# mfouda/epsilon

Hardware: AMD Instinct MI355X
Metric: ADMM iters/sec, dense Lasso 1e4x5e4 (higher is better)
Workload: dtype f32

## Files before the change

### epsilon_amd/csrc/capi.cc

```cpp
#include "../../include/epsilon_hip.h"

#include <algorithm>
#include <cmath>
#include <cstdio>
#include <cstdlib>
#include <cstring>
#include <map>
#include <memory>
#include <set>
#include <string>
#include <vector>

#include "admm.h"
#include "block.h"
#include "comm.h"
#include "kernels.h"
#include "linear_map.h"
#include "wire.h"

using namespace eps;

struct eps_result {
  std::string status;
  std::vector<std::string> ids;
  std::vector<HostArray> values;
};

struct eps_solver {
  std::shared_ptr<DataMap> data;
  std::unique_ptr<Solver> solver;
// ... 263 lines not shown
    } else if (std::strcmp(key, "fused") == 0) {
      setenv("EPSILON_HIP_FUSED", value, 1);
    } else if (std::strcmp(key, "batch_wide") == 0) {
      if (std::strcmp(value, "0") != 0 && std::strcmp(value, "1") != 0)
        EPS_FATAL("batch_wide must be 0 or 1, got " << value);
      setenv("EPSILON_HIP_BATCH_WIDE", value, 1);
    } else if (std::strcmp(key, "fused_matrix") == 0) {
      bool ok = false;
      for (const char* v : {"0", "pass", "wide", "auto"}) ok = ok || std::strcmp(value, v) == 0;
      if (!ok) EPS_FATAL("fused_matrix must be 0, pass, wide or auto, got " << value);
      setenv("EPSILON_HIP_FUSED_MATRIX", value, 1);
    } else if (std::strcmp(key, "fused_zero") == 0) {
      if (std::strcmp(value, "0") != 0 && std::strcmp(value, "auto") != 0)
        EPS_FATAL("fused_zero must be 0 or auto, got " << value);
      setenv("EPSILON_HIP_FUSED_ZERO", value, 1);
    } else if (std::strcmp(key, "refine") == 0) {
      if (std::strcmp(value, "auto") == 0) unsetenv("EPSILON_HIP_REFINE");
      else setenv("EPSILON_HIP_REFINE", value, 1);
    } else {
      EPS_FATAL("unknown option " << key);
    }
  });
}

int eps_device_count(void) {
  int count = 0;
  if (hipGetDeviceCount(&count) != hipSuccess) {
    (void)hipGetLastError();
    return 0;
  }
// ... 467 lines not shown
    const void* src = device_ptr;
    if (src == nullptr) {
      own = Synthetic(static_cast<int64_t>(bytes / 4), F32, 1.0);
      src = own.data();
    }
    EPS_HIP(hipDeviceSynchronize());
    DVec dst;
    if (mode == 2) dst = DVec::Empty(static_cast<int64_t>(bytes / 4), F32);
    if (grid <= 0) grid = 2048;
    DVec scratch = DVec::Empty(grid, F32);
    *ms_avg = TimeLaunches(iters, [&] {
      k::StreamProbe(mode, src, mode == 2 ? dst.data() : nullptr, static_cast<int64_t>(bytes),
                     scratch.as<float>(), grid);
    });
    (void)rt;
  });
}

int eps_bench_gemm(int trans_a, int trans_b, int64_t M, int64_t N, int64_t K, int lower_only,
                   int iters, double* ms_avg) {
  return Guard([&] {
    const DType dt = ConfiguredDType();
    const bool rnd = std::getenv("EPSILON_HIP_BENCH_RANDOM") != nullptr;
    auto operand = [&](int64_t count, uint64_t seed) {
      if (!rnd) return Synthetic(count, dt, 1.0);
      DVec v = DVec::Empty(count, dt);
      k::FillHash(v, seed);
      return v;
    };
    DVec A = operand(M * K, 0xA11CEull);
// ... 328 lines not shown
```

### epsilon_amd/csrc/fused_route.cc

```cpp
#include "fused_route.h"

#include <algorithm>
#include <cmath>
#include <cstdlib>
#include <cstring>
#include <map>

#include "admm.h"
#include "comm.h"
#include "kernels.h"

namespace eps {
namespace {


template <class Record>
void SetThreshold(Record* s, const ScaledZoneDesc& z, double a1) {
  s->alpha_vec = z.alpha_vec;
  s->beta_vec = z.beta_vec;
  s->Bs = z.Bs;
  s->Cs = z.Cs;
  s->a1 = a1;
  s->lam = z.lam;
  s->alpha = z.alpha;
// ... 72 lines not shown
  for (const StateSlice& s : table) s.home->Set(s.key, s.v);
}
std::vector<BlockVector*> Homes(const MultiBlockParts& a) {
  std::vector<BlockVector*> h = {&a.u};
  for (auto* c : {&a.x, &a.y, &a.y_prev})
    for (BlockVector& v : *c) h.push_back(&v);
  return h;
}

bool FusedDisabled() {
  const char* env = std::getenv("EPSILON_HIP_FUSED");
  return env && env[0] == '0';
}

int BatchWideMin();

constexpr int64_t kMatrixFusedMinRows = 256;

enum MatrixRoute { kMatrixOff, kMatrixAuto, kMatrixPass, kMatrixWide };
MatrixRoute FusedMatrixMode() {
  const char* e = std::getenv("EPSILON_HIP_FUSED_MATRIX");
  if (e == nullptr || std::strcmp(e, "auto") == 0) return kMatrixAuto;
  if (std::strcmp(e, "0") == 0) return kMatrixOff;
  if (std::strcmp(e, "pass") == 0) return kMatrixPass;
  if (std::strcmp(e, "wide") == 0) return kMatrixWide;
  EPS_FATAL("fused_matrix must be 0, pass, wide or auto, got " << e);
}

constexpr int64_t kZeroFusedMinRows = 256;

// ... 68 lines not shown
  DVec state_all, snapshot;
  DVec norm_work;
  int norm_slot = 0;
  bool whiten = false;
  double wscale = 1;
  DVec X, Ahat, rhat;
  k::LassoFusedArgs pass;
  int64_t cols = 1;
  bool group = false;
  int64_t group_rows = 0;
  bool wide = false;
  bool rhs_aligned = true;
  std::vector<k::LassoInstance> members;
  DVec table;
  WideSweep ws;

  bool Enable(const MultiBlockParts& a) {
    if (FusedDisabled() || a.prox.size() != 2 || a.num_constraints != 1 || !a.b.data().empty()) return false;
    const ShardSpec& sh = ShardSpec::Get();
    if (sh.active() && sh.consensus_terms()) return false;
    if (!a.prox[0]->DescribeLeastSquares(&ls)) return false;
    cols = ls.cols;
    const MatrixRoute matrix_mode = cols > 1 ? FusedMatrixMode() : kMatrixAuto;
    if (cols > 1 && (matrix_mode == kMatrixOff || sh.active())) return false;
    if (!a.prox[1]->DescribeScaledZone(&sz)) {
      GroupNorm2Desc gn;
      if (cols == 1 || !a.prox[1]->DescribeGroupNorm2(&gn) || gn.cols != cols) return false;
      group = true;
      group_rows = gn.rows;
      sz = ScaledZoneDesc();
// ... 198 lines not shown
    } else if (cols == 1) {
      inv.Apply();
    } else if (inv.packed.n > 0) {
      k::SymvPackedBatch(m, inv.D->scale(), inv.packed, table, static_cast<int>(cols), inv.work);
    } else {
      for (int64_t c = 0; c < cols; ++c) inv.Column(c).Apply();
    }
  }

  void BuildPass() {
    const DenseMatrixImpl& L = *ls.L_arg_var;
    pass.m = m;
    pass.n = n;
    pass.lda = whiten ? m : L.rows();
    pass.A = whiten ? Ahat : L.data();
    k::LassoInstance& s = pass.inst;
    s.w = w;
    s.tpart = tpart;
    s.p = whiten ? w : p;
    s.rhs = whiten ? rhat : ls.rhs_arg;
    s.kappa = -L.scale() * (whiten ? wscale : 1.0);
    s.pkappa = -L.scale();
    SetThreshold(&s, sz, a1);
    if (cols == 1) return;
    members.assign(static_cast<size_t>(cols), s);
    rhs_aligned = true;
    for (int64_t c = 0; c < cols; ++c) {
      k::LassoInstance& mb = members[static_cast<size_t>(c)];
      auto col = [&](const DVec& v, int64_t len) { return v.n > 0 ? v.Slice(c * len, len) : v; };
      mb.w = col(s.w, m);
// ... 16 lines not shown
    const int K = static_cast<int>(cols);
    const double* group_lam = group ? &sz.lam : nullptr;
    if (wide) {
      constexpr int PW = WideSweep::PW;
      for (int first = 0; first < K; first += PW) {
        const int nk = std::min(PW, K - first);
        const uint64_t live = nk == 64 ? ~uint64_t(0) : (uint64_t(1) << nk) - 1;
        const int64_t off = static_cast<int64_t>(first) * m;
        ws.Run(table, first, nk, live, w.Slice(off, ws.panel_len), whiten ? DVec() : p.Slice(off, ws.panel_len),
               group_lam);
      }
      return;
    }
    const int width = k::LassoBatchWidth(m, n, dt);
    for (int first = 0; first < K; first += width)
      k::LassoBatchPass(m, n, pass.lda, pass.A, table, first, std::min(width, K - first), group_lam);
    k::ReducePartialsBatch(m, grid, table, K, dt, rhs_aligned);
    if (!whiten) ApplyInverseFixed();
  }

  void Sweep() override {
    if (cols > 1) {
      MatrixSweep();
    } else if (use_peer) {
      pass.epoch = Runtime::Get().peer()->view().epoch;
      k::LassoFusedPass(pass);
      ForwardTailPeer();
    } else {
      k::LassoFusedPass(pass);
      ForwardTail(true);
    }
// ... 151 lines not shown
      return &views[first];
    };
    grid = k::LassoFusedGrid(m, n, dt);
    w = DVec::Zeros(m, dt);
    p = DVec::Zeros(m, dt);
    tpart = DVec::Empty(static_cast<int64_t>(grid) * m, dt);
    inv.Init(zp.Dinv_arg, m, p, w, a.shared_cache);
    {
      const StateSlice* sn = side(n, zp.x_constraint_key, ix, sx.var_key, zp.x_key, &state_n);
      pass.m = m;
      pass.n = n;
      pass.lda = L.rows();
      pass.A = L.data();
      pass.chain = 2;
      pass.e0 = sn[6].v;
      k::LassoInstance& s = pass.inst;
      s.w = w;
      s.tpart = tpart;
      s.p = p;
      s.rhs = zp.rhs_arg;
      s.u = sn[0].v;
      s.x1 = sn[1].v;
      s.x0 = sn[2].v;
      s.y1 = sn[3].v;
      s.y0 = sn[4].v;
      s.y1prev = sn[5].v;
      s.kappa = s.pkappa = -L.scale();
      SetThreshold(&s, sx, ax);
    }
    if (has_z) {
// ... 87 lines not shown
    for (BlockVector* home : {&a.x, &a.z, &a.u, &a.z_prev})
      for (const std::string& key : {ls.var_key, sz.var_key})
        views.push_back({home, key, DVec::Zeros(n, dt), home != &a.z_prev});
    const DVec &x0 = views[0].v, &x1 = views[1].v, &z0 = views[2].v, &z1 = views[3].v, &u0 = views[4].v,
               &u1 = views[5].v, &z0p = views[6].v, &z1p = views[7].v;
    p = DVec::Zeros(m, dt);
    w = DVec::Zeros(m, dt);
    grid = k::LassoFusedGrid(m, n, dt);
    tpart = DVec::Empty(static_cast<int64_t>(grid) * m, dt);
    pass.m = m;
    pass.n = n;
    pass.lda = L.rows();
    pass.A = L.data();
    pass.chain = 1;
    pass.a0 = a0;
    pass.e0 = u1;
    pass.e1 = z1p;
    k::LassoInstance& s = pass.inst;
    s.w = w;
    s.tpart = tpart;
    s.u = u0;
    s.x0 = x0;
    s.x1 = x1;
    s.y0 = z0;
    s.y1 = z1;
    s.y1prev = z0p;
    s.p = p;
    s.rhs = ls.rhs_arg;
    s.kappa = s.pkappa = -L.scale();
    SetThreshold(&s, sz, a1);
// ... 10 lines not shown
    k::LassoFusedPass(pass);
    k::ReducePartials(m, grid, tpart, pass.inst.pkappa, 0.0, p, ls.rhs_arg.n != 0 ? &ls.rhs_arg : nullptr);
    ls.Dinv_arg->Apply(1.0, p, 0.0, w);
  }
};

template <class Route, class Parts>
std::unique_ptr<FusedRoute> Recognise(const Parts& parts) {
  std::unique_ptr<Route> r(new Route);
  if (!r->Enable(parts)) return nullptr;
  return std::unique_ptr<FusedRoute>(std::move(r));
}

}

std::unique_ptr<FusedRoute> RecogniseMultiBlockRoute(const MultiBlockParts& parts) {
  const bool zero = FusedZeroAuto();
  if (auto r = Recognise<LassoRoute>(parts)) return r;
  return zero ? Recognise<ZeroRoute>(parts) : nullptr;
}

std::unique_ptr<FusedRoute> RecogniseTwoBlockRoute(const TwoBlockParts& parts) {
  return Recognise<TwoBlockRoute>(parts);
}

namespace {

struct BatchMember {
  Solver* solver;
  LassoRoute* route;
// ... 33 lines not shown
void RunFusedGroup(const Group& g) {
  const double t0 = Now();
  const LassoRoute& lead = *g[0].route;
  const DType dt = lead.dt;
  SetCurrentDType(dt);
  const int64_t m = lead.m, n = lead.n;
  const int width = k::LassoBatchWidth(m, n, dt);
  const DVec& P = lead.inv.packed;
  bool rhs_aligned = true;
  for (const BatchMember& b : g) {
    const DVec& rhs = b.route->pass.inst.rhs;
    if (rhs.n > 0) rhs_aligned = rhs_aligned && reinterpret_cast<uintptr_t>(rhs.data()) % 16 == 0;
  }
  const int K = static_cast<int>(g.size());
  DVec symv_work = P.n > 0 ? DVec::Empty(K * k::SymvWorkspace(m), dt) : DVec();

  std::vector<int> active(K);
  for (int i = 0; i < K; ++i) active[i] = i;
  DVec table;
  auto upload = [&] {
    std::vector<const k::LassoInstance*> v;
    for (int i : active) v.push_back(&g[i].route->pass.inst);
    k::LassoBatchUpload(v, dt, &table);
  };
  upload();
  auto sweep = [&] {
    const int na = static_cast<int>(active.size());
    for (int first = 0; first < na; first += width)
      k::LassoBatchPass(m, n, lead.pass.lda, lead.pass.A, table, first, std::min(width, na - first));
    k::ReducePartialsBatch(m, lead.grid, table, na, dt, rhs_aligned);
    if (lead.whiten) {
    } else if (P.n > 0) {
      k::SymvPackedBatch(m, lead.inv.D->scale(), P, table, na, symv_work);
    } else {
      for (int i : active) g[i].route->inv.Apply();
    }
  };
  RunGroupSchedule(g, t0, &active, sweep, [&](const std::vector<int>&) {
    if (!active.empty()) upload();
  });
}

bool BatchWideEnabled() {
  const char* e = std::getenv("EPSILON_HIP_BATCH_WIDE");
// ... 96 lines not shown
```

### epsilon_amd/csrc/fused_route.h

```cpp
#pragma once

#include <memory>
#include <vector>

#include "block.h"
#include "prox.h"

namespace eps {

class FusedRoute {
 public:
  virtual ~FusedRoute() {}
  virtual void Sweep() = 0;

  virtual bool HasCheck() const { return false; }
  virtual bool PipelineChecks() const { return false; }
  virtual void LaunchNorms() {}
  struct Check {
    double r = 0, s = 0;
    double max_norm = 0;
    double atu = 0;
  };
  virtual Check FinishCheck() { return Check(); }
  virtual void SaveSnapshot() {}
// ... 9 lines not shown
  const BlockVector& b;
  const std::vector<std::unique_ptr<ProxOperator>>& prox;
  DataMap* data;
  OpCache* shared_cache;
  BlockVector& u;
  std::vector<BlockVector>&x, &y, &y_prev;
};
struct TwoBlockParts {
  int num_constraints;
  const AffineOperator& constr_H;
  const std::vector<std::unique_ptr<ProxOperator>>& prox;
  DataMap* data;
  BlockVector &x, &z, &u, &z_prev;
};

std::unique_ptr<FusedRoute> RecogniseMultiBlockRoute(const MultiBlockParts& parts);
std::unique_ptr<FusedRoute> RecogniseTwoBlockRoute(const TwoBlockParts& parts);

}
```

### epsilon_amd/csrc/kernels.h

```cpp
#pragma once

#include "device.h"

namespace eps {
struct PeerView;
namespace k {

void Fill(const DVec& y, double v);
void Copy(const DVec& dst, const DVec& src);
void FillHash(const DVec& y, uint64_t seed);
void Axpby(const DVec& y, double a, const DVec& x, double b);
void DiagMul(const DVec& y, double a, const DVec& d, const DVec& x, double b);
void ConvertFromF64(const DVec& dst, const double* src_dev);
void ConvertToF64(double* dst_dev, const DVec& src);
void ConvertFromF32(const DVec& dst, const float* src_dev);

void SumSq(const DVec& x, double* slot, bool accumulate);
void SumSqDiff(const DVec& x, const DVec& y, double* slot, bool accumulate);
void Dot(const DVec& x, const DVec& y, double* slot, bool accumulate);

void Gemv(bool trans, int64_t rows, int64_t cols, double alpha, const DVec& A, int64_t lda,
          const DVec& x, double beta, const DVec& y);

void Symv(int64_t n, double alpha, const DVec& S, int64_t lds, const DVec& x, double beta,
// ... 14 lines not shown
  DVec alpha_vec, beta_vec;
  DVec p, rhs;
  double kappa = 0;
  double Bs = 0, Cs = 0, a1 = 0;
  double lam = 0, alpha = 1, beta = 1, M = 0;
  double pkappa = 0;
};
struct LassoFusedArgs {
  int64_t m = 0, n = 0, lda = 0;
  DVec A;
  LassoInstance inst;
  unsigned* epoch = nullptr;
  int chain = 0;
  double a0 = 1;
  DVec e0, e1;
};

enum SmoothFn { SMOOTH_EXP, SMOOTH_LOGISTIC, SMOOTH_NEG_ENTR, SMOOTH_INV_POS, SMOOTH_NEG_LOG };

struct ZeroRowsArgs {
  int64_t m = 0;
  int nparts = 0;
  DVec w, tpart, r, rhs, g;
  DVec u, z, zq, yz, yq, yzprev, yqprev;
  DVec alpha_vec, beta_vec;
  double e = 0, pkappa = 0;
  double Bs = 0, Cs = 0, a1 = 0, lam = 0, alpha = 1, beta = 1, M = 0;
  bool smooth = false;
  SmoothFn fn = SMOOTH_LOGISTIC;
  DVec hs, hys, hv;
};
void ZeroFusedRows(const ZeroRowsArgs& args);
void ZeroSmoothHead(const ZeroRowsArgs& args);
bool LassoFusedSupported(int64_t m, int64_t n, const DVec& A, int64_t lda);
int LassoFusedGrid(int64_t m, int64_t n, DType dt = F32);
int LassoFusedBlock(int64_t m, int64_t n, DType dt);
void LassoFusedPass(const LassoFusedArgs& args);
void LassoFusedNorms(const DVec& u, const DVec& y0, const DVec& y1, const DVec& y1prev, double* out6,
                     const DVec& work, const unsigned* peer_err = nullptr);

template <class T> struct LassoBatchInst {
  const T* w;
  T* tpart;
  T* u; T* x0; T* x1; T* y0; T* y1; T* y1prev;
  const T* alpha_v;
  const T* beta_v;
  T* p;
  const T* rhs;
  T kappa, Bs, Cs, a1, lam, alpha, beta, M;
  T pkappa;
};
int LassoBatchWidth(int64_t m, int64_t n, DType dt);
void LassoBatchUpload(const std::vector<const LassoInstance*>& members, DType dt, DVec* table);
void LassoBatchPass(int64_t m, int64_t n, int64_t lda, const DVec& A, const DVec& table, int first,
                    int count, const double* group_lam = nullptr);
void ReducePartialsBatch(int64_t m, int nparts, const DVec& table, int count, DType dt,
                         bool rhs_aligned);
void SymvPackedBatch(int64_t m, double alpha, const DVec& P, const DVec& table, int count,
                     const DVec& work);

constexpr int kLassoWidePanel = 64;
bool LassoWideSupported(int64_t m, int64_t n, const DVec& A, int64_t lda);
int LassoWideSlabs(int64_t m, int64_t n);
void LassoWideBack(int64_t m, int64_t n, int64_t lda, const DVec& A, const DVec& table, int first, int nk,
                   uint64_t active, const DVec& W, int64_t ldw, const DVec& V, int64_t ldv,
                   const double* group_lam = nullptr);
void LassoWideForward(int64_t m, int64_t n, int64_t lda, const DVec& A, int nk, const DVec& V, int64_t ldv,
                      const DVec& T, int64_t ldt);
void LassoWideReduce(int64_t m, int64_t n, const DVec& table, int first, int nk, uint64_t active, const DVec& T,
                     int64_t ldt);
// ... 14 lines not shown
                 bool lower_only = false, int64_t outer = 1, int64_t sA2 = 0, int64_t sB2 = 0);
void SymmetrizeFromLower(const DVec& C, int64_t n, int64_t ldc);
bool GemmSplitF16(bool transA, bool transB, int64_t M, int64_t N, int64_t K, double alpha, const DVec& A,
                  int64_t lda, const DVec& B, int64_t ldb, double beta, const DVec& C, int64_t ldc,
                  bool lower_only);
bool GemmF64Pipe(bool transA, bool transB, int64_t M, int64_t N, int64_t K, double alpha, const DVec& A,
                 int64_t lda, int64_t sA, const DVec& B, int64_t ldb, int64_t sB, double beta,
                 const DVec& C, int64_t ldc, int64_t sC, int64_t n1, int64_t batch, bool lower_only,
                 int64_t sA2, int64_t sB2);
bool GemmSplitF16KRange(int kmode, int64_t M, int64_t N, int64_t K, double alpha, const DVec& A, int64_t lda,
                        const DVec& B, int64_t ldb, const DVec& C, int64_t ldc);
bool SyrkSplitF16LowerTriangular(int64_t n, const DVec& X, int64_t ldx, const DVec& C, int64_t ldc);
bool MultiGemv(bool transA, int64_t M, int64_t N, int64_t K, double alpha, const DVec& A, int64_t lda,
               const DVec& B, int64_t ldb, double beta, const DVec& C, int64_t ldc);
void StreamProbe(int mode, const void* src, void* dst, int64_t bytes, float* scratch, int grid);

void MatCopy(bool trans, int64_t rows, int64_t cols, double alpha, const DVec& src,
             int64_t lds, const DVec& dst);
void AddDiag(const DVec& W, int64_t n, int64_t ld, double alpha, const DVec* d);
void ColAbsSums(const DVec& A, int64_t rows, int64_t cols, int64_t lda, double* colsum_dev);
void ScaleByInvNorm(const DVec& y, const DVec& x, const double* normsq_dev);
void KronDense(const DVec& dst, const DVec& A, int64_t mA, int64_t nA, const DVec& B,
               int64_t mB, int64_t nB);

void SpdInverseInPlace(const DVec& W, int64_t n, DVec* factor_inverse = nullptr);
void SetPotrfForm(int form);
void SpdInverseColumns(const DVec& W, int64_t n, int64_t lo, int64_t cnt, const DVec& Out);

struct ScaledZoneArgs {
  double lam = 0, alpha = 1, beta = 1, M = 0, C = 0;
// ... 56 lines not shown
```

### epsilon_amd/csrc/kernels_fused.hip

```cpp
#include <hip/hip_runtime.h>

#include <cstdlib>
#include <type_traits>

#include "kernels.h"
#include "kernels_fused_chain.h"

namespace eps {
namespace k {

namespace {

constexpr int kBlock = 256;

template <class T, int NR, int BS, int MODE>
__global__ __launch_bounds__(BS, 2) void LassoFusedStreamKernelT(
    int64_t m, int64_t n, const T* __restrict__ A, int64_t lda, const T* __restrict__ w,
    FusedScalarsT<T> c, T* u, T* x0, T* x1, T* y0, T* y1, T* y1prev, T* __restrict__ tpart,
    unsigned* epoch, T* e0, T* e1) {
  typedef typename Chunk<T>::V V;
  constexpr int R = Chunk<T>::R;
  __shared__ T red[2][BS / 64];
  if (epoch != nullptr && blockIdx.x == 0 && threadIdx.x == 0) *epoch += 1u;
  const int tid = threadIdx.x, lane = tid & 63, wave = tid >> 6;
  const V zero = T(0);
  V wv[NR], tp[NR];
  int64_t row[NR];
#pragma unroll
  for (int q = 0; q < NR; ++q) {
    row[q] = (static_cast<int64_t>(q) * BS + tid) * R;
    wv[q] = row[q] < m ? *reinterpret_cast<const V*>(w + row[q]) : zero;
    tp[q] = zero;
  }
  const int64_t npairs = (n + 1) / 2;
  auto column = [&](int64_t step) -> int64_t {
    const int64_t jp = blockIdx.x + (step >> 1) * gridDim.x;
    const int64_t j = 2 * jp + (step & 1);
    return (jp < npairs && j < n) ? j : -1;
  };
  auto load = [&](V (&a)[NR], int64_t j) {
    const T* cp = A + j * lda;
#pragma unroll
    for (int q = 0; q < NR; ++q) {
      if (row[q] < m) a[q] = __builtin_nontemporal_load(reinterpret_cast<const V*>(cp + row[q]));
      else a[q] = zero;
    }
  };
  V cur[NR], nxt[NR];
  int64_t step = 0;
  int64_t j = column(0);
  if (j >= 0) load(cur, j);
  int par = 0;
  while (j >= 0) {
    int64_t jn = column(step + 1);
    if (jn < 0 && ((step + 1) & 1)) jn = column(step + 2);
    const int64_t step_n = (jn >= 0 && column(step + 1) < 0) ? step + 2 : step + 1;
    if (jn >= 0) load(nxt, jn);
    const T uj = u[j], y0j = y0[j], y1j = y1[j];
    T u1j = T(0);
// ... 63 lines not shown
  T* out = tpart + static_cast<int64_t>(blockIdx.x) * m;
#pragma unroll
  for (int q = 0; q < NR; ++q)
    if (row[q] < m) *reinterpret_cast<V*>(out + row[q]) = tp[q];
}

template <class T, int NR, int BS>
void LaunchFused(const LassoFusedArgs& a, int grid) {
  const LassoBatchInst<T> i = Narrow<T>(a.inst);
  T* e0 = a.chain != 0 ? a.e0.as<T>() : nullptr;
  T* e1 = a.chain == 1 ? a.e1.as<T>() : nullptr;
  hipLaunchKernelGGL(
      (a.chain == 1 ? LassoFusedStreamKernelT<T, NR, BS, 1>
                    : a.chain == 2 ? LassoFusedStreamKernelT<T, NR, BS, 2> : LassoFusedStreamKernelT<T, NR, BS, 0>),
      dim3(grid), dim3(BS), 0, Runtime::Get().stream(), a.m, a.n, a.A.as<T>(), a.lda, i.w,
      ScalarsOf<T>(i, a.a0, a.inst.a1), i.u, i.x0, i.x1, i.y0, i.y1, i.y1prev, i.tpart, a.epoch, e0, e1);
}

template <class T>
void LaunchFusedT(const LassoFusedArgs& a, int grid, int block) {
  const int64_t need = (a.m + Chunk<T>::R * block - 1) / (Chunk<T>::R * block);
  if (block == 256) {
    if (need <= 1) LaunchFused<T, 1, 256>(a, grid);
    else if (need <= 2) LaunchFused<T, 2, 256>(a, grid);
    else if (need <= 4) LaunchFused<T, 4, 256>(a, grid);
    else if (need <= 8) LaunchFused<T, 8, 256>(a, grid);
    else LaunchFused<T, 10, 256>(a, grid);
    return;
  }
  if constexpr (std::is_same<T, float>::value) {
    if (need <= 2) return LaunchFused<T, 2, 512>(a, grid);
// ... 236 lines not shown

int LassoFusedGrid(int64_t m, int64_t n, DType dt) {
  int64_t npairs = (n + 1) / 2;
  const int64_t rows_per_chunk = dt == F32 ? 4 : 2;
  const bool one_per_cu = LassoFusedBlock(m, n, dt) == 512 && m > 512 * 5 * rows_per_chunk;
  int64_t g = one_per_cu ? 256 : 512;
  static const char* env = std::getenv("EPSILON_HIP_FUSED_GRID");
  if (env && std::atoi(env) > 0) g = std::atoi(env);
  if (g > npairs) g = npairs;
  if (g < 1) g = 1;
  const int64_t per = (npairs + g - 1) / g;
  g = (npairs + per - 1) / per;
  return static_cast<int>(g < 1 ? 1 : g);
}

void LassoFusedPass(const LassoFusedArgs& a) {
  EPS_CHECK(LassoFusedSupported(a.m, a.n, a.A, a.lda));
  const DType dt = a.A.dt;
  const LassoInstance& s = a.inst;
  EPS_CHECK(s.w.n == a.m && s.w.dt == dt);
  for (const DVec* v : {&s.u, &s.x0, &s.x1, &s.y0, &s.y1, &s.y1prev})
    EPS_CHECK(v->n == a.n && v->dt == dt);
  for (const DVec* v : {&s.alpha_vec, &s.beta_vec})
    if (v->n > 0) EPS_CHECK(v->n == a.n && v->dt == dt);
  if (a.chain == 1) EPS_CHECK(a.e0.n == a.n && a.e1.n == a.n && a.e0.dt == dt && a.e1.dt == dt);
  if (a.chain == 2) EPS_CHECK(a.e0.n == a.n && a.e0.dt == dt);
  const int grid = LassoFusedGrid(a.m, a.n, dt);
  const int block = LassoFusedBlock(a.m, a.n, dt);
  EPS_CHECK(s.tpart.n >= static_cast<int64_t>(grid) * a.m && s.tpart.dt == dt);
  EPS_CHECK(reinterpret_cast<uintptr_t>(s.w.data()) % 16 == 0 &&
            reinterpret_cast<uintptr_t>(s.tpart.data()) % 16 == 0);
  ProfScope prof(a.chain == 2 ? "zero_fused" : "lasso_fused", a.m, a.n);
  if (dt == F32) LaunchFusedT<float>(a, grid, block);
  else LaunchFusedT<double>(a, grid, block);
  EPS_HIP(hipGetLastError());
}

}
}
```

### epsilon_amd/csrc/kernels_fused_batch.hip

```cpp
#include <hip/hip_runtime.h>

#include <vector>

#include "kernels.h"
#include "kernels_fused_chain.h"

namespace eps {
namespace k {

namespace {

constexpr int kBlock = 256;

template <class T, int NR, int KB, bool GROUP>
__global__ __launch_bounds__(kBlock) void LassoBatchStreamKernel(int64_t m, int64_t n, const T* __restrict__ A,
                                                                 int64_t lda,
                                                                 const LassoBatchInst<T>* __restrict__ tab,
                                                                 int nk, double glam) {
  typedef typename Chunk<T>::V V;
  constexpr int R = Chunk<T>::R;
  __shared__ T red[2][KB][kBlock / 64];
  const int tid = threadIdx.x, lane = tid & 63, wave = tid >> 6;
  V zero;
#pragma unroll
  for (int r = 0; r < R; ++r) zero[r] = T(0);
  V wv[KB][NR], tp[KB][NR];
  int64_t row[NR];
#pragma unroll
  for (int q = 0; q < NR; ++q) row[q] = (static_cast<int64_t>(q) * kBlock + tid) * R;
#pragma unroll
  for (int i = 0; i < KB; ++i) {
#pragma unroll
    for (int q = 0; q < NR; ++q) {
      wv[i][q] = (i < nk && row[q] < m) ? *reinterpret_cast<const V*>(tab[i].w + row[q]) : zero;
      tp[i][q] = zero;
    }
  }
  const int64_t npairs = (n + 1) / 2;
  auto column = [&](int64_t step) -> int64_t {
    const int64_t jp = blockIdx.x + (step >> 1) * gridDim.x;
    const int64_t j = 2 * jp + (step & 1);
    return (jp < npairs && j < n) ? j : -1;
  };
  auto load = [&](V (&a)[NR], int64_t j) {
    const T* cp = A + j * lda;
#pragma unroll
    for (int q = 0; q < NR; ++q)
      a[q] = row[q] < m ? __builtin_nontemporal_load(reinterpret_cast<const V*>(cp + row[q])) : zero;
  };
  V cur[NR], nxt[NR];
  int64_t step = 0;
  int64_t j = column(0);
  if (j >= 0) load(cur, j);
  int par = 0;
  while (j >= 0) {
    int64_t jn = column(step + 1);
    if (jn < 0 && ((step + 1) & 1)) jn = column(step + 2);
    const int64_t step_n = (jn >= 0 && column(step + 1) < 0) ? step + 2 : step + 1;
    if (jn >= 0) load(nxt, jn);
    T uj[KB], y0j[KB], y1j[KB];
#pragma unroll
    for (int i = 0; i < KB; ++i) {
      if (i >= nk) continue;
// ... 100 lines not shown
    for (int q = 0; q < NR; ++q)
      if (row[q] < m) *reinterpret_cast<V*>(out + row[q]) = tp[i][q];
  }
}

int ChunksPerThread(int64_t m, DType dt) {
  const int64_t rows = dt == F32 ? 4 : 2;
  const int64_t need = (m + rows * kBlock - 1) / (rows * kBlock);
  return need <= 1 ? 1 : need <= 2 ? 2 : need <= 4 ? 4 : need <= 8 ? 8 : 10;
}

constexpr int WidthFor(int nr) { return nr <= 2 ? 8 : nr <= 4 ? 6 : nr <= 8 ? 5 : 4; }

template <class T, int NR>
void LaunchBatch(int grid, int64_t m, int64_t n, const T* A, int64_t lda, const LassoBatchInst<T>* tab, int nk,
                 const double* glam) {
  if (glam != nullptr)
    hipLaunchKernelGGL((LassoBatchStreamKernel<T, NR, WidthFor(NR), true>), dim3(grid), dim3(kBlock), 0,
                       Runtime::Get().stream(), m, n, A, lda, tab, nk, *glam);
  else
    hipLaunchKernelGGL((LassoBatchStreamKernel<T, NR, WidthFor(NR), false>), dim3(grid), dim3(kBlock), 0,
                       Runtime::Get().stream(), m, n, A, lda, tab, nk, 0.0);
}

template <class T>
void LaunchBatchT(int nr, int grid, int64_t m, int64_t n, const T* A, int64_t lda, const LassoBatchInst<T>* tab,
                  int nk, const double* glam) {
  switch (nr) {
    case 1: LaunchBatch<T, 1>(grid, m, n, A, lda, tab, nk, glam); break;
    case 2: LaunchBatch<T, 2>(grid, m, n, A, lda, tab, nk, glam); break;
    case 4: LaunchBatch<T, 4>(grid, m, n, A, lda, tab, nk, glam); break;
    case 8: LaunchBatch<T, 8>(grid, m, n, A, lda, tab, nk, glam); break;
    default: LaunchBatch<T, 10>(grid, m, n, A, lda, tab, nk, glam); break;
  }
}

template <class T>
void UploadT(const std::vector<const LassoInstance*>& members, DVec* table) {
  std::vector<LassoBatchInst<T>> host;
  host.reserve(members.size());
  for (const LassoInstance* s : members) host.push_back(Narrow<T>(*s));
  const size_t bytes = host.size() * sizeof(LassoBatchInst<T>);
  const int64_t words = static_cast<int64_t>((bytes + 7) / 8);
  if (table->n < words || table->dt != F64) *table = DVec::Empty(words < 1 ? 1 : words, F64);
  if (bytes == 0) return;
  Runtime& rt = Runtime::Get();
  EPS_HIP(hipMemcpyAsync(table->data(), host.data(), bytes, hipMemcpyHostToDevice, rt.stream()));
  rt.Sync();
// ... 3 lines not shown

int LassoBatchWidth(int64_t m, int64_t n, DType dt) {
  if (LassoFusedBlock(m, n, dt) != kBlock) return 0;
  return WidthFor(ChunksPerThread(m, dt));
}

void LassoBatchUpload(const std::vector<const LassoInstance*>& members, DType dt, DVec* table) {
  for (const LassoInstance* s : members)
    for (const DVec* v : {&s->w, &s->tpart, &s->u, &s->x0, &s->x1, &s->y0, &s->y1, &s->y1prev, &s->p})
      EPS_CHECK(v->dt == dt && v->n > 0);
  if (dt == F32) UploadT<float>(members, table);
  else UploadT<double>(members, table);
}

void LassoBatchPass(int64_t m, int64_t n, int64_t lda, const DVec& A, const DVec& table, int first, int count,
                    const double* group_lam) {
  const DType dt = A.dt;
  EPS_CHECK(LassoFusedSupported(m, n, A, lda));
  const int width = LassoBatchWidth(m, n, dt);
  EPS_CHECK_MSG(width > 0 && count >= 1 && count <= width,
                "batched fused pass: " << count << " instances, width " << width);
  const int grid = LassoFusedGrid(m, n, dt);
  const int nr = ChunksPerThread(m, dt);
  ProfScope prof("batch_fused_pass", m, n);
  if (dt == F32)
    LaunchBatchT<float>(nr, grid, m, n, A.as<float>(), lda,
                        reinterpret_cast<const LassoBatchInst<float>*>(table.as<char>()) + first, count, group_lam);
  else
    LaunchBatchT<double>(nr, grid, m, n, A.as<double>(), lda,
                         reinterpret_cast<const LassoBatchInst<double>*>(table.as<char>()) + first, count, group_lam);
  EPS_HIP(hipGetLastError());
}

}
}
```

### epsilon_amd/csrc/kernels_fused_chain.h

```cpp
#pragma once

#include <hip/hip_runtime.h>

#include <type_traits>

#include "kernels.h"
#include "kernels_smooth_fn.h"

namespace eps {
namespace k {
namespace {

template <class T> struct Chunk;
template <> struct Chunk<float> {
  static constexpr int R = 4;
  typedef float V __attribute__((ext_vector_type(4)));
};
template <> struct Chunk<double> {
  static constexpr int R = 2;
  typedef double V __attribute__((ext_vector_type(2)));
};

template <class T> struct FusedScalarsT {
  T kappa;
  T Bs, Cs, a1, lam, alpha, beta, M;
  T a0, inv_aa;
  const T* alpha_v;
  const T* beta_v;
};

template <class T> LassoBatchInst<T> Narrow(const LassoInstance& s) {
  LassoBatchInst<T> d;
  d.w = s.w.as<T>();
  d.tpart = s.tpart.as<T>();
  d.u = s.u.as<T>();
  d.x0 = s.x0.as<T>();
// ... 136 lines not shown
```

### epsilon_amd/csrc/kernels_vec.hip

```cpp
#include <hip/hip_runtime.h>

#include "kernels.h"

namespace eps {
namespace k {

namespace {

constexpr int kBlock = 256;
constexpr int kMaxGrid = 2048;

template <class T> struct Pack;
template <> struct Pack<float> { using type = float4; static constexpr int V = 4; };
template <> struct Pack<double> { using type = double2; static constexpr int V = 2; };

inline bool Aligned16(const void* p) { return (reinterpret_cast<uintptr_t>(p) & 15) == 0; }

inline int GridFor(int64_t work_items) {
  int64_t g = (work_items + kBlock - 1) / kBlock;
  if (g < 1) g = 1;
  if (g > kMaxGrid) g = kMaxGrid;
  return static_cast<int>(g);
}

// ... 443 lines not shown
  }
  for (; i < n4; i += stride) {
    const f32x4_probe v = p[i];
    acc += v.x + v.y + v.z + v.w;
  }
  __shared__ float red[256];
  red[threadIdx.x] = acc;
  __syncthreads();
  for (int off = 128; off > 0; off >>= 1) {
    if (static_cast<int>(threadIdx.x) < off) red[threadIdx.x] += red[threadIdx.x + off];
    __syncthreads();
  }
  if (threadIdx.x == 0) out[blockIdx.x] = red[0];
}

__global__ __launch_bounds__(256) void StreamCopyKernel(const f32x4_probe* __restrict__ src,
                                                        f32x4_probe* __restrict__ dst, int64_t n4) {
  const int64_t stride = static_cast<int64_t>(gridDim.x) * 256;
  for (int64_t i = static_cast<int64_t>(blockIdx.x) * 256 + threadIdx.x; i < n4; i += stride)
    dst[i] = src[i];
}
}

void StreamProbe(int mode, const void* src, void* dst, int64_t bytes, float* scratch, int grid) {
  hipStream_t s = Runtime::Get().stream();
  const int64_t n4 = bytes / 16;
  const auto* p = static_cast<const f32x4_probe*>(src);
  if (mode == 0)
    hipLaunchKernelGGL(StreamReadKernel<true>, dim3(grid), dim3(256), 0, s, p, n4, scratch);
  else if (mode == 1)
    hipLaunchKernelGGL(StreamReadKernel<false>, dim3(grid), dim3(256), 0, s, p, n4, scratch);
  else
    hipLaunchKernelGGL(StreamCopyKernel, dim3(grid), dim3(256), 0, s, p, static_cast<f32x4_probe*>(dst), n4);
}

}
}
```

### include/epsilon_hip.h

```cpp
#ifndef EPSILON_HIP_H_
#define EPSILON_HIP_H_

#include <stddef.h>
#include <stdint.h>

#ifdef __cplusplus
extern "C" {
#endif

enum {
  EPS_BLOB_HOST = 0,
  EPS_BLOB_DEVICE_F32 = 1,
  EPS_BLOB_DEVICE_F64 = 2
};
typedef struct eps_blob {
  const char* key;
  const void* ptr;
  size_t len;
  int kind;
} eps_blob;

typedef struct eps_param {
  const char* id;
  const void* constant_proto;
// ... 58 lines not shown
int eps_profile_reset(void);
int eps_profile_dump(char* buf, size_t cap);


int eps_linear_map_apply(const void* linear_map, size_t len, const eps_blob* data, size_t ndata,
                         int transpose, const double* x, size_t nx, double* y, size_t ny);
int eps_linear_map_binary(char op, const void* a, size_t a_len, int ta, const void* b,
                          size_t b_len, int tb, const eps_blob* data, size_t ndata,
                          int* result_type, int64_t* m, int64_t* n, double* dense,
                          size_t dense_capacity);
int eps_linear_map_inverse(const void* linear_map, size_t len, const eps_blob* data,
                           size_t ndata, double* dense, size_t dense_capacity);
int eps_bench_gemv(int trans, int64_t rows, int64_t cols, int iters, double* ms_avg);
int eps_bench_stream(const void* device_ptr, size_t bytes, int mode, int grid, int iters,
                     double* ms_avg);
int eps_bench_gemm(int trans_a, int trans_b, int64_t M, int64_t N, int64_t K, int lower_only,
                   int iters, double* ms_avg);
int eps_bench_spd_inverse(int64_t n, int iters, double* ms_avg);
int eps_bench_spd_inverse_columns(int64_t n, int64_t cnt, int iters, double* ms_avg);
int eps_test_spd_inverse_repeat(int64_t n, int form_a, int form_b, double* diff_fro, double* norm_fro);

typedef struct eps_block {
  const char* row;
  const char* col;
  const void* linear_map;
  size_t len;
} eps_block;
int eps_test_block_solve(const char* mode, const eps_block* blocks, size_t nblocks,
                         const eps_blob* data, size_t ndata, const eps_blob* rhs, size_t nrhs,
                         const char* const* keys, size_t nkeys, eps_result** out);
// ... 23 lines not shown
```

Before: 3095.

## Keep a budgeted slice of the Lasso matrix cache-resident in fused passes

```diff
diff --git a/epsilon_amd/csrc/capi.cc b/epsilon_amd/csrc/capi.cc
--- a/epsilon_amd/csrc/capi.cc
+++ b/epsilon_amd/csrc/capi.cc
@@ -14,6 +14,7 @@
 #include "admm.h"
 #include "block.h"
 #include "comm.h"
+#include "fused_route.h"
 #include "kernels.h"
 #include "linear_map.h"
 #include "wire.h"
@@ -307,6 +308,9 @@
       if (std::strcmp(value, "0") != 0 && std::strcmp(value, "auto") != 0)
         EPS_FATAL("fused_zero must be 0 or auto, got " << value);
       setenv("EPSILON_HIP_FUSED_ZERO", value, 1);
+    } else if (std::strcmp(key, "fused_resident") == 0) {
+      (void)ParseFusedResident(value);
+      setenv("EPSILON_HIP_FUSED_RESIDENT_KB", value, 1);
     } else if (std::strcmp(key, "refine") == 0) {
       if (std::strcmp(value, "auto") == 0) unsetenv("EPSILON_HIP_REFINE");
       else setenv("EPSILON_HIP_REFINE", value, 1);
@@ -804,6 +808,49 @@
                      scratch.as<float>(), grid);
     });
     (void)rt;
+  });
+}
+
+int eps_bench_stream_resident(const void* device_ptr, size_t bytes, size_t resident_bytes, int grid, int iters,
+                              double* ms_avg) {
+  return Guard([&] {
+    const size_t column = 40000;
+    EPS_CHECK_MSG(bytes >= column && resident_bytes <= bytes && iters >= 1 && ms_avg != nullptr,
+                  "eps_bench_stream_resident: bad arguments");
+    DVec own;
+    const void* src = device_ptr;
+    if (src == nullptr) {
+      own = Synthetic(static_cast<int64_t>(bytes / 4), F32, 1.0);
+      src = own.data();
+    }
+    EPS_HIP(hipDeviceSynchronize());
+    if (grid <= 0) grid = 2048;
+    DVec scratch = DVec::Empty(grid, F32);
+    const int64_t per_column = static_cast<int64_t>(resident_bytes / (bytes / column)) / 16 * 16;
+    *ms_avg = TimeLaunches(iters, [&] {
+      k::StreamResidentProbe(src, static_cast<int64_t>(bytes), per_column, scratch.as<float>(), grid);
+    });
+  });
+}
+
+int eps_fused_residency(int64_t m, int64_t n, int f64, int64_t budget_bytes, int* qfull, int64_t* jcut,
+                        int64_t* resident_bytes) {
+  return Guard([&] {
+    EPS_CHECK_MSG(m >= 1 && n >= 1 && qfull != nullptr && jcut != nullptr && resident_bytes != nullptr,
+                  "eps_fused_residency: bad arguments");
+    const k::FusedResidency r = k::LassoFusedResidency(m, n, f64 ? F64 : F32, budget_bytes);
+    *qfull = r.qfull;
+    *jcut = r.jcut;
+    *resident_bytes = r.bytes;
+  });
+}
+
+int eps_fused_residency_last(int* qfull, int64_t* jcut) {
+  return Guard([&] {
+    EPS_CHECK_MSG(qfull != nullptr && jcut != nullptr, "eps_fused_residency_last: bad arguments");
+    const k::FusedResidency r = k::LastFusedResidency();
+    *qfull = r.qfull;
+    *jcut = r.jcut;
   });
 }
 
diff --git a/epsilon_amd/csrc/fused_route.cc b/epsilon_amd/csrc/fused_route.cc
--- a/epsilon_amd/csrc/fused_route.cc
+++ b/epsilon_amd/csrc/fused_route.cc
@@ -110,6 +110,19 @@
 }
 
 int BatchWideMin();
+
+constexpr int64_t kResidentLimitBytes = int64_t(224) << 20;
+
+int64_t FusedResidentOption() {
+  const char* e = std::getenv("EPSILON_HIP_FUSED_RESIDENT_KB");
+  return e == nullptr ? -1 : ParseFusedResident(e);
+}
+
+k::FusedResidency ResidentShare(int64_t m, int64_t n, DType dt, int64_t touched, bool auto_on) {
+  int64_t budget = FusedResidentOption();
+  if (budget < 0) budget = auto_on ? std::max<int64_t>(0, kResidentLimitBytes - touched) : 0;
+  return k::LassoFusedResidency(m, n, dt, budget);
+}
 
 constexpr int64_t kMatrixFusedMinRows = 256;
 
@@ -208,6 +221,14 @@
   std::vector<k::LassoInstance> members;
   DVec table;
   WideSweep ws;
+  k::FusedResidency res;
+
+  k::FusedResidency Residency(int64_t count) const {
+    if (sharded || use_peer || wide || ShardSpec::Get().active()) return k::FusedResidency();
+    const int64_t sz = dt == F32 ? 4 : 8;
+    const int64_t touched = (count * (static_cast<int64_t>(grid) * m + 6 * n + 2 * m) + (whiten ? 0 : m * m)) * sz;
+    return ResidentShare(m, n, dt, touched, count == 1 && cols == 1);
+  }
 
   bool Enable(const MultiBlockParts& a) {
     if (FusedDisabled() || a.prox.size() != 2 || a.num_constraints != 1 || !a.b.data().empty()) return false;
@@ -436,6 +457,9 @@
     pass.n = n;
     pass.lda = whiten ? m : L.rows();
     pass.A = whiten ? Ahat : L.data();
+    res = Residency(cols);
+    pass.qfull = res.qfull;
+    pass.jcut = res.jcut;
     k::LassoInstance& s = pass.inst;
     s.w = w;
     s.tpart = tpart;
@@ -482,7 +506,7 @@
     }
     const int width = k::LassoBatchWidth(m, n, dt);
     for (int first = 0; first < K; first += width)
-      k::LassoBatchPass(m, n, pass.lda, pass.A, table, first, std::min(width, K - first), group_lam);
+      k::LassoBatchPass(m, n, pass.lda, pass.A, table, first, std::min(width, K - first), group_lam, res);
     k::ReducePartialsBatch(m, grid, table, K, dt, rhs_aligned);
     if (!whiten) ApplyInverseFixed();
   }
@@ -664,6 +688,11 @@
       pass.A = L.data();
       pass.chain = 2;
       pass.e0 = sn[6].v;
+      const int64_t sz = dt == F32 ? 4 : 8;
+      const k::FusedResidency res =
+          ResidentShare(m, n, dt, (static_cast<int64_t>(grid) * m + 7 * (n + m) + 2 * m + m * m) * sz, false);
+      pass.qfull = res.qfull;
+      pass.jcut = res.jcut;
       k::LassoInstance& s = pass.inst;
       s.w = w;
       s.tpart = tpart;
@@ -781,6 +810,13 @@
     pass.A = L.data();
     pass.chain = 1;
     pass.a0 = a0;
+    {
+      const int64_t sz = dt == F32 ? 4 : 8;
+      const k::FusedResidency res =
+          ResidentShare(m, n, dt, (static_cast<int64_t>(grid) * m + 8 * n + 2 * m + m * m) * sz, false);
+      pass.qfull = res.qfull;
+      pass.jcut = res.jcut;
+    }
     pass.e0 = u1;
     pass.e1 = z1p;
     k::LassoInstance& s = pass.inst;
@@ -821,6 +857,19 @@
 
 }
 
+int64_t ParseFusedResident(const char* value) {
+  if (std::strcmp(value, "auto") == 0) return -1;
+  const int64_t cap = int64_t(1) << 40;
+  int64_t kb = 0;
+  bool ok = value[0] != '\0';
+  for (const char* c = value; ok && *c != '\0'; ++c) {
+    ok = *c >= '0' && *c <= '9';
+    if (ok) kb = std::min(cap, kb * 10 + (*c - '0'));
+  }
+  if (!ok) EPS_FATAL("fused_resident must be auto or a number of KiB, got " << value);
+  return kb * 1024;
+}
+
 std::unique_ptr<FusedRoute> RecogniseMultiBlockRoute(const MultiBlockParts& parts) {
   const bool zero = FusedZeroAuto();
   if (auto r = Recognise<LassoRoute>(parts)) return r;
@@ -884,6 +933,7 @@
   }
   const int K = static_cast<int>(g.size());
   DVec symv_work = P.n > 0 ? DVec::Empty(K * k::SymvWorkspace(m), dt) : DVec();
+  const k::FusedResidency res = lead.Residency(K);
 
   std::vector<int> active(K);
   for (int i = 0; i < K; ++i) active[i] = i;
@@ -897,7 +947,7 @@
   auto sweep = [&] {
     const int na = static_cast<int>(active.size());
     for (int first = 0; first < na; first += width)
-      k::LassoBatchPass(m, n, lead.pass.lda, lead.pass.A, table, first, std::min(width, na - first));
+      k::LassoBatchPass(m, n, lead.pass.lda, lead.pass.A, table, first, std::min(width, na - first), nullptr, res);
     k::ReducePartialsBatch(m, lead.grid, table, na, dt, rhs_aligned);
     if (lead.whiten) {
     } else if (P.n > 0) {
diff --git a/epsilon_amd/csrc/fused_route.h b/epsilon_amd/csrc/fused_route.h
--- a/epsilon_amd/csrc/fused_route.h
+++ b/epsilon_amd/csrc/fused_route.h
@@ -47,6 +47,8 @@
   BlockVector &x, &z, &u, &z_prev;
 };
 
+int64_t ParseFusedResident(const char* value);
+
 std::unique_ptr<FusedRoute> RecogniseMultiBlockRoute(const MultiBlockParts& parts);
 std::unique_ptr<FusedRoute> RecogniseTwoBlockRoute(const TwoBlockParts& parts);
 
diff --git a/epsilon_amd/csrc/kernels.h b/epsilon_amd/csrc/kernels.h
--- a/epsilon_amd/csrc/kernels.h
+++ b/epsilon_amd/csrc/kernels.h
@@ -52,6 +52,8 @@
   int chain = 0;
   double a0 = 1;
   DVec e0, e1;
+  int qfull = 0;
+  int64_t jcut = 0;
 };
 
 enum SmoothFn { SMOOTH_EXP, SMOOTH_LOGISTIC, SMOOTH_NEG_ENTR, SMOOTH_INV_POS, SMOOTH_NEG_LOG };
@@ -73,6 +75,14 @@
 bool LassoFusedSupported(int64_t m, int64_t n, const DVec& A, int64_t lda);
 int LassoFusedGrid(int64_t m, int64_t n, DType dt = F32);
 int LassoFusedBlock(int64_t m, int64_t n, DType dt);
+struct FusedResidency {
+  int qfull = 0;
+  int64_t jcut = 0;
+  int64_t bytes = 0;
+};
+FusedResidency LassoFusedResidency(int64_t m, int64_t n, DType dt, int64_t budget);
+FusedResidency LastFusedResidency();
+void NoteFusedResidency(int qfull, int64_t jcut);
 void LassoFusedPass(const LassoFusedArgs& args);
 void LassoFusedNorms(const DVec& u, const DVec& y0, const DVec& y1, const DVec& y1prev, double* out6,
                      const DVec& work, const unsigned* peer_err = nullptr);
@@ -91,7 +101,7 @@
 int LassoBatchWidth(int64_t m, int64_t n, DType dt);
 void LassoBatchUpload(const std::vector<const LassoInstance*>& members, DType dt, DVec* table);
 void LassoBatchPass(int64_t m, int64_t n, int64_t lda, const DVec& A, const DVec& table, int first,
-                    int count, const double* group_lam = nullptr);
+                    int count, const double* group_lam = nullptr, const FusedResidency& res = FusedResidency());
 void ReducePartialsBatch(int64_t m, int nparts, const DVec& table, int count, DType dt,
                          bool rhs_aligned);
 void SymvPackedBatch(int64_t m, double alpha, const DVec& P, const DVec& table, int count,
@@ -136,6 +146,7 @@
 bool MultiGemv(bool transA, int64_t M, int64_t N, int64_t K, double alpha, const DVec& A, int64_t lda,
                const DVec& B, int64_t ldb, double beta, const DVec& C, int64_t ldc);
 void StreamProbe(int mode, const void* src, void* dst, int64_t bytes, float* scratch, int grid);
+void StreamResidentProbe(const void* src, int64_t bytes, int64_t resident_per_column, float* scratch, int grid);
 
 void MatCopy(bool trans, int64_t rows, int64_t cols, double alpha, const DVec& src,
              int64_t lds, const DVec& dst);
diff --git a/epsilon_amd/csrc/kernels_fused.hip b/epsilon_amd/csrc/kernels_fused.hip
--- a/epsilon_amd/csrc/kernels_fused.hip
+++ b/epsilon_amd/csrc/kernels_fused.hip
@@ -1,5 +1,6 @@
 #include <hip/hip_runtime.h>
 
+#include <algorithm>
 #include <cstdlib>
 #include <type_traits>
 
@@ -17,7 +18,7 @@
 __global__ __launch_bounds__(BS, 2) void LassoFusedStreamKernelT(
     int64_t m, int64_t n, const T* __restrict__ A, int64_t lda, const T* __restrict__ w,
     FusedScalarsT<T> c, T* u, T* x0, T* x1, T* y0, T* y1, T* y1prev, T* __restrict__ tpart,
-    unsigned* epoch, T* e0, T* e1) {
+    unsigned* epoch, T* e0, T* e1, int qfull, int64_t jcut) {
   typedef typename Chunk<T>::V V;
   constexpr int R = Chunk<T>::R;
   __shared__ T red[2][BS / 64];
@@ -40,9 +41,10 @@
   };
   auto load = [&](V (&a)[NR], int64_t j) {
     const T* cp = A + j * lda;
+    const int nres = qfull + (j < jcut ? 1 : 0);
 #pragma unroll
     for (int q = 0; q < NR; ++q) {
-      if (row[q] < m) a[q] = __builtin_nontemporal_load(reinterpret_cast<const V*>(cp + row[q]));
+      if (row[q] < m) a[q] = LoadMatrixChunk<T>(cp + row[q], q < nres);
       else a[q] = zero;
     }
   };
@@ -136,7 +138,8 @@
       (a.chain == 1 ? LassoFusedStreamKernelT<T, NR, BS, 1>
                     : a.chain == 2 ? LassoFusedStreamKernelT<T, NR, BS, 2> : LassoFusedStreamKernelT<T, NR, BS, 0>),
       dim3(grid), dim3(BS), 0, Runtime::Get().stream(), a.m, a.n, a.A.as<T>(), a.lda, i.w,
-      ScalarsOf<T>(i, a.a0, a.inst.a1), i.u, i.x0, i.x1, i.y0, i.y1, i.y1prev, i.tpart, a.epoch, e0, e1);
+      ScalarsOf<T>(i, a.a0, a.inst.a1), i.u, i.x0, i.x1, i.y0, i.y1, i.y1prev, i.tpart, a.epoch, e0, e1,
+      a.qfull, a.jcut);
 }
 
 template <class T>
@@ -403,8 +406,39 @@
   return static_cast<int>(g < 1 ? 1 : g);
 }
 
+FusedResidency LassoFusedResidency(int64_t m, int64_t n, DType dt, int64_t budget) {
+  FusedResidency r;
+  if (budget <= 0 || m < 1 || n < 1) return r;
+  const int64_t elem = dt == F32 ? 4 : 8;
+  const int64_t chunk_rows = static_cast<int64_t>(LassoFusedBlock(m, n, dt)) * (16 / elem);
+  const int64_t nchunks = (m + chunk_rows - 1) / chunk_rows;
+  for (int64_t q = 0; q < nchunks; ++q) {
+    const int64_t piece = std::min(chunk_rows, m - q * chunk_rows) * elem;
+    const int64_t left = budget - r.bytes;
+    if (left / piece >= n) {
+      r.bytes += piece * n;
+      r.qfull = static_cast<int>(q + 1);
+      continue;
+    }
+    r.jcut = left / piece;
+    r.bytes += piece * r.jcut;
+    break;
+  }
+  return r;
+}
+
+namespace {
+FusedResidency g_last_residency;
+}
+FusedResidency LastFusedResidency() { return g_last_residency; }
+void NoteFusedResidency(int qfull, int64_t jcut) {
+  g_last_residency.qfull = qfull;
+  g_last_residency.jcut = jcut;
+}
+
 void LassoFusedPass(const LassoFusedArgs& a) {
   EPS_CHECK(LassoFusedSupported(a.m, a.n, a.A, a.lda));
+  EPS_CHECK(a.qfull >= 0 && a.jcut >= 0 && a.jcut <= a.n);
   const DType dt = a.A.dt;
   const LassoInstance& s = a.inst;
   EPS_CHECK(s.w.n == a.m && s.w.dt == dt);
@@ -420,6 +454,7 @@
   EPS_CHECK(reinterpret_cast<uintptr_t>(s.w.data()) % 16 == 0 &&
             reinterpret_cast<uintptr_t>(s.tpart.data()) % 16 == 0);
   ProfScope prof(a.chain == 2 ? "zero_fused" : "lasso_fused", a.m, a.n);
+  NoteFusedResidency(a.qfull, a.jcut);
   if (dt == F32) LaunchFusedT<float>(a, grid, block);
   else LaunchFusedT<double>(a, grid, block);
   EPS_HIP(hipGetLastError());
diff --git a/epsilon_amd/csrc/kernels_fused_batch.hip b/epsilon_amd/csrc/kernels_fused_batch.hip
--- a/epsilon_amd/csrc/kernels_fused_batch.hip
+++ b/epsilon_amd/csrc/kernels_fused_batch.hip
@@ -16,14 +16,13 @@
 __global__ __launch_bounds__(kBlock) void LassoBatchStreamKernel(int64_t m, int64_t n, const T* __restrict__ A,
                                                                  int64_t lda,
                                                                  const LassoBatchInst<T>* __restrict__ tab,
-                                                                 int nk, double glam) {
+                                                                 int nk, double glam, int qfull,
+                                                                 int64_t jcut) {
   typedef typename Chunk<T>::V V;
   constexpr int R = Chunk<T>::R;
   __shared__ T red[2][KB][kBlock / 64];
   const int tid = threadIdx.x, lane = tid & 63, wave = tid >> 6;
-  V zero;
-#pragma unroll
-  for (int r = 0; r < R; ++r) zero[r] = T(0);
+  const V zero = T(0);
   V wv[KB][NR], tp[KB][NR];
   int64_t row[NR];
 #pragma unroll
@@ -44,9 +43,12 @@
   };
   auto load = [&](V (&a)[NR], int64_t j) {
     const T* cp = A + j * lda;
-#pragma unroll
-    for (int q = 0; q < NR; ++q)
-      a[q] = row[q] < m ? __builtin_nontemporal_load(reinterpret_cast<const V*>(cp + row[q])) : zero;
+    const int nres = qfull + (j < jcut ? 1 : 0);
+#pragma unroll
+    for (int q = 0; q < NR; ++q) {
+      if (row[q] < m) a[q] = LoadMatrixChunk<T>(cp + row[q], q < nres);
+      else a[q] = zero;
+    }
   };
   V cur[NR], nxt[NR];
   int64_t step = 0;
@@ -177,24 +179,24 @@
 
 template <class T, int NR>
 void LaunchBatch(int grid, int64_t m, int64_t n, const T* A, int64_t lda, const LassoBatchInst<T>* tab, int nk,
-                 const double* glam) {
+                 const double* glam, const FusedResidency& res) {
   if (glam != nullptr)
     hipLaunchKernelGGL((LassoBatchStreamKernel<T, NR, WidthFor(NR), true>), dim3(grid), dim3(kBlock), 0,
-                       Runtime::Get().stream(), m, n, A, lda, tab, nk, *glam);
+                       Runtime::Get().stream(), m, n, A, lda, tab, nk, *glam, res.qfull, res.jcut);
   else
     hipLaunchKernelGGL((LassoBatchStreamKernel<T, NR, WidthFor(NR), false>), dim3(grid), dim3(kBlock), 0,
-                       Runtime::Get().stream(), m, n, A, lda, tab, nk, 0.0);
+                       Runtime::Get().stream(), m, n, A, lda, tab, nk, 0.0, res.qfull, res.jcut);
 }
 
 template <class T>
 void LaunchBatchT(int nr, int grid, int64_t m, int64_t n, const T* A, int64_t lda, const LassoBatchInst<T>* tab,
-                  int nk, const double* glam) {
+                  int nk, const double* glam, const FusedResidency& res) {
   switch (nr) {
-    case 1: LaunchBatch<T, 1>(grid, m, n, A, lda, tab, nk, glam); break;
-    case 2: LaunchBatch<T, 2>(grid, m, n, A, lda, tab, nk, glam); break;
-    case 4: LaunchBatch<T, 4>(grid, m, n, A, lda, tab, nk, glam); break;
-    case 8: LaunchBatch<T, 8>(grid, m, n, A, lda, tab, nk, glam); break;
-    default: LaunchBatch<T, 10>(grid, m, n, A, lda, tab, nk, glam); break;
+    case 1: LaunchBatch<T, 1>(grid, m, n, A, lda, tab, nk, glam, res); break;
+    case 2: LaunchBatch<T, 2>(grid, m, n, A, lda, tab, nk, glam, res); break;
+    case 4: LaunchBatch<T, 4>(grid, m, n, A, lda, tab, nk, glam, res); break;
+    case 8: LaunchBatch<T, 8>(grid, m, n, A, lda, tab, nk, glam, res); break;
+    default: LaunchBatch<T, 10>(grid, m, n, A, lda, tab, nk, glam, res); break;
   }
 }
 
@@ -228,21 +230,23 @@
 }
 
 void LassoBatchPass(int64_t m, int64_t n, int64_t lda, const DVec& A, const DVec& table, int first, int count,
-                    const double* group_lam) {
+                    const double* group_lam, const FusedResidency& res) {
   const DType dt = A.dt;
   EPS_CHECK(LassoFusedSupported(m, n, A, lda));
+  EPS_CHECK(res.qfull >= 0 && res.jcut >= 0 && res.jcut <= n);
   const int width = LassoBatchWidth(m, n, dt);
   EPS_CHECK_MSG(width > 0 && count >= 1 && count <= width,
                 "batched fused pass: " << count << " instances, width " << width);
   const int grid = LassoFusedGrid(m, n, dt);
   const int nr = ChunksPerThread(m, dt);
   ProfScope prof("batch_fused_pass", m, n);
+  NoteFusedResidency(res.qfull, res.jcut);
   if (dt == F32)
     LaunchBatchT<float>(nr, grid, m, n, A.as<float>(), lda,
-                        reinterpret_cast<const LassoBatchInst<float>*>(table.as<char>()) + first, count, group_lam);
+                        reinterpret_cast<const LassoBatchInst<float>*>(table.as<char>()) + first, count, group_lam, res);
   else
     LaunchBatchT<double>(nr, grid, m, n, A.as<double>(), lda,
-                         reinterpret_cast<const LassoBatchInst<double>*>(table.as<char>()) + first, count, group_lam);
+                         reinterpret_cast<const LassoBatchInst<double>*>(table.as<char>()) + first, count, group_lam, res);
   EPS_HIP(hipGetLastError());
 }
 
diff --git a/epsilon_amd/csrc/kernels_fused_chain.h b/epsilon_amd/csrc/kernels_fused_chain.h
--- a/epsilon_amd/csrc/kernels_fused_chain.h
+++ b/epsilon_amd/csrc/kernels_fused_chain.h
@@ -20,6 +20,13 @@
   static constexpr int R = 2;
   typedef double V __attribute__((ext_vector_type(2)));
 };
+
+template <class T> __device__ inline typename Chunk<T>::V LoadMatrixChunk(const T* p, bool resident) {
+  typedef typename Chunk<T>::V V;
+  typedef const V __attribute__((address_space(4))) * ConstV;
+  if (resident) return *(ConstV)(p);
+  return __builtin_nontemporal_load(reinterpret_cast<const V*>(p));
+}
 
 template <class T> struct FusedScalarsT {
   T kappa;
diff --git a/epsilon_amd/csrc/kernels_vec.hip b/epsilon_amd/csrc/kernels_vec.hip
--- a/epsilon_amd/csrc/kernels_vec.hip
+++ b/epsilon_amd/csrc/kernels_vec.hip
@@ -481,6 +481,37 @@
   if (threadIdx.x == 0) out[blockIdx.x] = red[0];
 }
 
+constexpr int kProbeColumn = 2500;
+
+__global__ __launch_bounds__(256) void StreamResidentKernel(const f32x4_probe* __restrict__ p, int64_t ncols,
+                                                            int rv, float* __restrict__ out) {
+  typedef const f32x4_probe __attribute__((address_space(4))) * ConstV;
+  constexpr int kPer = (kProbeColumn + 255) / 256;
+  const int tid = threadIdx.x;
+  float acc = 0.f;
+  for (int64_t c = blockIdx.x; c < ncols; c += gridDim.x) {
+    const f32x4_probe* cp = p + c * kProbeColumn;
+    f32x4_probe v[kPer];
+#pragma unroll
+    for (int q = 0; q < kPer; ++q) {
+      const int i = q * 256 + tid;
+      if (i >= kProbeColumn) v[q] = 0.f;
+      else if (i < rv) v[q] = *(ConstV)(cp + i);
+      else v[q] = __builtin_nontemporal_load(cp + i);
+    }
+#pragma unroll
+    for (int q = 0; q < kPer; ++q) acc += (v[q].x + v[q].y) + (v[q].z + v[q].w);
+  }
+  __shared__ float red[256];
+  red[tid] = acc;
+  __syncthreads();
+  for (int off = 128; off > 0; off >>= 1) {
+    if (tid < off) red[tid] += red[tid + off];
+    __syncthreads();
+  }
+  if (tid == 0) out[blockIdx.x] = red[0];
+}
+
 __global__ __launch_bounds__(256) void StreamCopyKernel(const f32x4_probe* __restrict__ src,
                                                         f32x4_probe* __restrict__ dst, int64_t n4) {
   const int64_t stride = static_cast<int64_t>(gridDim.x) * 256;
@@ -501,5 +532,15 @@
     hipLaunchKernelGGL(StreamCopyKernel, dim3(grid), dim3(256), 0, s, p, static_cast<f32x4_probe*>(dst), n4);
 }
 
-}
-}
+void StreamResidentProbe(const void* src, int64_t bytes, int64_t resident_per_column, float* scratch, int grid) {
+  const int64_t ncols = bytes / (16 * kProbeColumn);
+  int64_t rv = resident_per_column / 16;
+  if (rv < 0) rv = 0;
+  if (rv > kProbeColumn) rv = kProbeColumn;
+  if (ncols < 1) return;
+  hipLaunchKernelGGL(StreamResidentKernel, dim3(grid), dim3(256), 0, Runtime::Get().stream(),
+                     static_cast<const f32x4_probe*>(src), ncols, static_cast<int>(rv), scratch);
+}
+
+}
+}
diff --git a/include/epsilon_hip.h b/include/epsilon_hip.h
--- a/include/epsilon_hip.h
+++ b/include/epsilon_hip.h
@@ -96,6 +96,11 @@
 int eps_bench_gemv(int trans, int64_t rows, int64_t cols, int iters, double* ms_avg);
 int eps_bench_stream(const void* device_ptr, size_t bytes, int mode, int grid, int iters,
                      double* ms_avg);
+int eps_bench_stream_resident(const void* device_ptr, size_t bytes, size_t resident_bytes, int grid,
+                              int iters, double* ms_avg);
+int eps_fused_residency(int64_t m, int64_t n, int f64, int64_t budget_bytes, int* qfull, int64_t* jcut,
+                        int64_t* resident_bytes);
+int eps_fused_residency_last(int* qfull, int64_t* jcut);
 int eps_bench_gemm(int trans_a, int trans_b, int64_t M, int64_t N, int64_t K, int lower_only,
                    int iters, double* ms_avg);
 int eps_bench_spd_inverse(int64_t n, int iters, double* ms_avg);
```

Result: faster. 3380 (median of 6 runs) (+9.2%).
